# taddallas/HMSC

Measured on AMD Instinct MI355X. Metric: Gibbs sweeps/sec + Beta ESS/sec at ny=10k, ns=1k, nf=10; 1/2/4/8 MI355X, higher is better.
Workload: dtype f64; 1 GPU; synthetic probit JSDM ny=10000 ns=1000 nc=20 nf=10, 1 sample-level random level, updater GammaEta=FALSE, record every sweep; ny=10000, ns=1000, nc=20, nf=10, parallelism=1 independent chains, one per GPU

## Files before the change

### hmsc_amd/csrc/z_kernel.h

```cpp
#pragma once
#include <hip/hip_runtime.h>
#include <stdint.h>

#include "common.h"
#include "rng.h"
#include "record.h"
#include "z_tables.h"

namespace hmsc {

constexpr int Z_NSEG = 4;
struct ZSeg {
  int n, t;
};

struct ZArgs {
  const double* XEta;
  int ny, K, ns_loc, sp0, nt;
  ZSeg seg[Z_NSEG];
#ifdef HMSC_STAMPS
  int stamp_by, stamp_chunk;
#endif
  const double* BL;
  const double* iSigma;
  const int8_t* Ycode;
  const uint64_t* Ybits;
  const double* Yval;
  const int* fam;
  const double* Tr;
  double* Z;
  double* XZ_part;
  double* ZTr_part;
  Key key;
  uint32_t iter;
  const uint32_t* iter_dev;
  int noise_zero;
  int zprev_is_e;
  int mask_na;
  unsigned long long* kt;
  int gred_y0, gred_groups, gred_ntile, gred_nf, gred_Kmax;
  const double* gred_part;
  const double* gred_XX;
  double* gred_G;
  const double* logtab;
  const double* ztab;
  int pack_row;
  PackArgs pack;
};

constexpr int ZT_I = 64;
constexpr int ZT_J = 32;
constexpr int KMAX_Z = 128;
constexpr int ZT_LD = 65;

typedef double d4 __attribute__((ext_vector_type(4)));

__device__ __forceinline__ d4 mfma_f64(double a, double b, d4 c) {
  return __builtin_amdgcn_mfma_f64_16x16x4f64(a, b, c, 0, 0, 0);
}

__device__ __forceinline__ void wave_lds_sync() {
  __builtin_amdgcn_fence(__ATOMIC_RELEASE, "wavefront");
  __builtin_amdgcn_wave_barrier();
  __builtin_amdgcn_fence(__ATOMIC_ACQUIRE, "wavefront");
}

template <int N>
__device__ __forceinline__ double row_ror(double v) {
  const long long b = __double_as_longlong(v);
  const int lo = __builtin_amdgcn_update_dpp(0, (int)b, 0x120 + N, 0xF, 0xF, false);
  const int hi = __builtin_amdgcn_update_dpp(0, (int)(b >> 32), 0x120 + N, 0xF, 0xF, false);
  return __longlong_as_double(((long long)hi << 32) | (unsigned int)lo);
}
__device__ __forceinline__ double row_sum16(double v) {
  v += row_ror<8>(v);
  v += row_ror<4>(v);
  v += row_ror<2>(v);
  v += row_ror<1>(v);
  return v;
}

__device__ __noinline__ double z_probit_draw(double e, double sd, double isd, int code, double u, int noise_zero) {
  const double sg = code == 0 ? -1.0 : 1.0;
  if (code < 0 && noise_zero) return e;
  const double alpha = code < 0 ? -INFINITY : -sg * e * isd;
  return e + sd * sg * trunc_normal_lower(alpha, u);
}

constexpr int ZLOG_N = 64;
constexpr int ZLOG_W = 2;
inline void z_log_table(double* t) {
  for (int j = 0; j < ZLOG_N; ++j) {
    const long double c = 1.0L + (2 * j + 1) / 128.0L;
    t[ZLOG_W * j] = (double)(1.0L / c);
    t[ZLOG_W * j + 1] = (double)logl(c);
  }
}
HMSC_TABLE double kLog1pSeries[5] = {1.0 / 5.0, -1.0 / 4.0, 1.0 / 3.0, -1.0 / 2.0, 1.0};
__device__ __forceinline__ double log_tab(double x, const double* tab) {
  const int e = __builtin_amdgcn_frexp_exp(x) - 1;
  const double m2 = 2.0 * __builtin_amdgcn_frexp_mant(x);
  uint64_t b;
  __builtin_memcpy(&b, &m2, 8);
  const uint32_t hi = (uint32_t)(b >> 32);
  const int j = (int)((hi >> 14) & 63u);
  const uint64_t cb = (uint64_t)((hi & 0xFFFFC000u) | 0x2000u) << 32;
  double c;
  __builtin_memcpy(&c, &cb, 8);
  const double* tj = tab + ZLOG_W * j;
  const double r = (m2 - c) * tj[0];
  double P = kLog1pSeries[0];
#pragma unroll
  for (int k = 1; k < 5; ++k) P = fma_sc(P, r, kLog1pSeries[k]);
  const double de = (double)e;
  return fma(de, 0.6931471803691238, tj[1]) + fma(r, P, de * 1.9082149292705877e-10);
}

struct ZPair {
  double z0, z1;
};

#ifndef ZT_Q_LD_DEF
#define ZT_Q_LD_DEF 10
#endif
constexpr int ZT_E_LD = 10, ZT_Q_LD = ZT_Q_LD_DEF;
constexpr int ZT_E_SEG = ZT_E_MAX * ZT_E_PER_UNIT, ZT_Q_SEG = ZT_Q_MAX * ZT_Q_PER_UNIT;
constexpr int ZT_X_N = 64;
constexpr int ZT_OFF_E = 0, ZT_OFF_Q = ZT_E_SEG * ZT_E_LD, ZT_OFF_X = ZT_OFF_Q + ZT_Q_SEG * ZT_Q_LD;
constexpr int ZT_DOUBLES = ZT_OFF_X + ZT_X_N;
static_assert(ZT_E_NC % 2 == 0 && ZT_Q_NC % 2 == 0 && ZT_E_LD % 2 == 0 && ZT_Q_LD % 2 == 0 && ZT_E_LD >= ZT_E_NC &&
                  ZT_Q_LD >= ZT_Q_NC,
              "16-byte rows");
inline void z_draw_tables(double* t) {
  for (int i = 0; i < ZT_DOUBLES; ++i) t[i] = 0.0;
  for (int j = 0; j < ZT_E_SEG; ++j)
    for (int k = 0; k < ZT_E_NC; ++k) t[ZT_OFF_E + ZT_E_LD * j + k] = kZtErfcx[ZT_E_NC * j + k];
  for (int j = 0; j < ZT_Q_SEG; ++j)
    for (int k = 0; k < ZT_Q_NC; ++k) t[ZT_OFF_Q + ZT_Q_LD * j + k] = kZtQnormF[ZT_Q_NC * j + k];
  for (int i = 0; i < ZT_X_N; ++i) t[ZT_OFF_X + i] = kZtExp2[i];
}
typedef double zt_d2 __attribute__((ext_vector_type(2)));

template <int NC>
__device__ __forceinline__ double zt_poly(const double* row, double d) {
  const zt_d2* r2 = (const zt_d2*)row;
  zt_d2 c[NC / 2];
#pragma unroll
  for (int k = 0; k < NC / 2; ++k) c[k] = r2[k];
  double v = c[0][0];
  v = fma(v, d, c[0][1]);
#pragma unroll
  for (int k = 1; k < NC / 2; ++k) {
    v = fma(v, d, c[k][0]);
    v = fma(v, d, c[k][1]);
  }
  return v;
}

HMSC_TABLE double kZtExpPoly[6] = {1.0 / 120.0, 1.0 / 24.0, 1.0 / 6.0, 0.5, 1.0, 1.0};
template <bool IN_RANGE = false>
__device__ __forceinline__ double zt_erfc(double a, const double* zt) {
  const int j = IN_RANGE ? (int)(a * (double)ZT_E_PER_UNIT) : min((int)(a * (double)ZT_E_PER_UNIT), ZT_E_SEG - 1);
  const double d = a - ((double)j + 0.5) * (1.0 / ZT_E_PER_UNIT);
  const double* row = IN_RANGE ? (const double*)((const char*)(zt + ZT_OFF_E) +
                                                 __umul24((unsigned int)j, (unsigned int)(ZT_E_LD * sizeof(double))))
                               : zt + ZT_OFF_E + ZT_E_LD * j;
  const double cx = zt_poly<ZT_E_NC>(row, d);
  const double hi = a * a, lo = fma(a, a, -hi);
  const double kf = __builtin_rint(hi * -92.33248261689366);
  double r = fma(kf, -0.01083042469326756, -hi);
  r = fma(kf, -2.9815858269852933e-12, r) - lo;
  double p = kZtExpPoly[0];
#pragma unroll
  for (int k = 1; k < 6; ++k) p = fma_sc(p, r, kZtExpPoly[k]);
  const int ki = (int)kf;
  return __builtin_ldexp(p * zt[ZT_OFF_X + (ki & 63)], ki >> 6) * cx;
}

__device__ __forceinline__ double zt_qnorm_w(double p, double w, const double* zt) {
  const int j = max(0, min((int)(w * (double)ZT_Q_PER_UNIT), ZT_Q_SEG - 1));
  const double d = w - ((double)j + 0.5) * (1.0 / ZT_Q_PER_UNIT);
  return (2.0 * p - 1.0) * zt_poly<ZT_Q_NC>(zt + ZT_OFF_Q + ZT_Q_LD * j, d);
}

__device__ __forceinline__ ZPair z_probit_pair_tab(double e0, double e1, double sd0, double sd1, double isd0,
                                                double isd1, int c0, int c1, double u0, double u1, int noise_zero,
                                                const double* ltab, const double* zt) {
  const double sg0 = c0 == 0 ? -1.0 : 1.0, sg1 = c1 == 0 ? -1.0 : 1.0;
  const double al0 = c0 < 0 ? -INFINITY : -sg0 * e0 * isd0;
  const double al1 = c1 < 0 ? -INFINITY : -sg1 * e1 * isd1;
  double q0, q1;
  if (al0 > 25.0 || al1 > 25.0) {
    q0 = -trunc_normal_lower(al0, u0);
    q1 = -trunc_normal_lower(al1, u1);
  } else {
    const double a0 = fmin(fabs(al0) * 0.7071067811865476, 17.99);
    const double a1 = fmin(fabs(al1) * 0.7071067811865476, 17.99);
    const double r0 = 0.5 * zt_erfc(a0, zt), r1 = 0.5 * zt_erfc(a1, zt);
    const double s0 = 1.0 - r0, s1 = 1.0 - r1;
    const double p0 = u0 * (al0 < 0.0 ? s0 : r0), pc0 = fma(u0, al0 < 0.0 ? r0 : s0, 1.0 - u0);
    const double p1 = u1 * (al1 < 0.0 ? s1 : r1), pc1 = fma(u1, al1 < 0.0 ? r1 : s1, 1.0 - u1);
    const double w0 = -log_tab(4.0 * p0 * pc0, ltab), w1 = -log_tab(4.0 * p1 * pc1, ltab);
    q0 = zt_qnorm_w(p0, w0, zt);
    q1 = zt_qnorm_w(p1, w1, zt);
    if (w0 >= (double)ZT_Q_MAX || w1 >= (double)ZT_Q_MAX) {
      if (w0 >= (double)ZT_Q_MAX) q0 = qnorm_as241_tail_pq_t(p0, pc0, kLogSeries);
      if (w1 >= (double)ZT_Q_MAX) q1 = qnorm_as241_tail_pq_t(p1, pc1, kLogSeries);
    }
  }
  ZPair z;
  z.z0 = (c0 < 0 && noise_zero) ? e0 : e0 - sd0 * sg0 * q0;
  z.z1 = (c1 < 0 && noise_zero) ? e1 : e1 - sd1 * sg1 * q1;
  return z;
}
__device__ __forceinline__ double z_flip(double x, uint32_t f) {
  return __hiloint2double(__double2hiint(x) ^ (int)f, __double2loint(x));
}
__device__ __forceinline__ ZPair z_probit_pair_lean(double e0, double e1, uint32_t f0, uint32_t f1, double u0,
                                                    double u1, const double* ltab, const double* zt) {
  const double al0 = z_flip(e0, f0), al1 = z_flip(e1, f1);
  double q0, q1;
  if (al0 > 25.0 || al1 > 25.0) {
    q0 = -trunc_normal_lower(al0, u0);
    q1 = -trunc_normal_lower(al1, u1);
  } else {
    const double a0 = fmin(fabs(al0) * 0.7071067811865476, 17.99);
    const double a1 = fmin(fabs(al1) * 0.7071067811865476, 17.99);
    const double r0 = 0.5 * zt_erfc<true>(a0, zt), r1 = 0.5 * zt_erfc<true>(a1, zt);
    const double s0 = 1.0 - r0, s1 = 1.0 - r1;
    const double p0 = u0 * (al0 < 0.0 ? s0 : r0), pc0 = fma(u0, al0 < 0.0 ? r0 : s0, 1.0 - u0);
    const double p1 = u1 * (al1 < 0.0 ? s1 : r1), pc1 = fma(u1, al1 < 0.0 ? r1 : s1, 1.0 - u1);
    const double w0 = -log_tab(4.0 * p0 * pc0, ltab), w1 = -log_tab(4.0 * p1 * pc1, ltab);
    q0 = zt_qnorm_w(p0, w0, zt);
    q1 = zt_qnorm_w(p1, w1, zt);
    if (w0 >= (double)ZT_Q_MAX || w1 >= (double)ZT_Q_MAX) {
      if (w0 >= (double)ZT_Q_MAX) q0 = qnorm_as241_tail_pq_t(p0, pc0, kLogSeries);
      if (w1 >= (double)ZT_Q_MAX) q1 = qnorm_as241_tail_pq_t(p1, pc1, kLogSeries);
    }
  }
  ZPair z;
  z.z0 = e0 + z_flip(q0, f0);
  z.z1 = e1 + z_flip(q1, f1);
  return z;
}
__device__ __forceinline__ ZPair z_probit_pair(double e0, double e1, double sd0, double sd1, double isd0, double isd1,
                                            int c0, int c1, double u0, double u1, int noise_zero,
                                            const double* ltab) {
  const double sg0 = c0 == 0 ? -1.0 : 1.0, sg1 = c1 == 0 ? -1.0 : 1.0;
  const double al0 = c0 < 0 ? -INFINITY : -sg0 * e0 * isd0;
  const double al1 = c1 < 0 ? -INFINITY : -sg1 * e1 * isd1;
  double q0, q1;
  if (al0 > 25.0 || al1 > 25.0) {
    q0 = -trunc_normal_lower(al0, u0);
    q1 = -trunc_normal_lower(al1, u1);
  } else {
    const double h0 = al0 * 0.7071067811865476, h1 = al1 * 0.7071067811865476;
    const double a0 = fmin(fabs(h0), 40.0), a1 = fmin(fabs(h1), 40.0);
    const double t0 = 2.0 * rcp_pos(2.0 + a0), t1 = 2.0 * rcp_pos(2.0 + a1);
    const double x0 = 2.0 * t0 - 1.0, x1 = 2.0 * t1 - 1.0;
    double g0 = kErfcPoly[0], g1 = kErfcPoly[0];
#pragma unroll
    for (int k = 1; k < ERFC_NC; ++k) {
      g0 = fma_sc(g0, x0, kErfcPoly[k]);
      g1 = fma_sc(g1, x1, kErfcPoly[k]);
    }
    const double r0 = t0 * exp_small(fma(-a0, a0, g0)), r1 = t1 * exp_small(fma(-a1, a1, g1));
    const double p0 = u0 * (0.5 * (h0 < 0.0 ? 2.0 - r0 : r0));
    const double p1 = u1 * (0.5 * (h1 < 0.0 ? 2.0 - r1 : r1));
    const double pc0 = h0 < 0.0 ? fma(u0, 0.5 * r0, 1.0 - u0) : 1.0 - p0;
    const double pc1 = h1 < 0.0 ? fma(u1, 0.5 * r1, 1.0 - u1) : 1.0 - p1;
    const double w0 = -log_tab(4.0 * p0 * pc0, ltab), w1 = -log_tab(4.0 * p1 * pc1, ltab);
    const double y0 = w0 - 3.125, y1 = w1 - 3.125;
    double F0 = kQnormA[0], F1 = kQnormA[0];
#pragma unroll
    for (int k = 1; k < QNA_NC; ++k) {
      F0 = fma_sc(F0, y0, kQnormA[k]);
      F1 = fma_sc(F1, y1, kQnormA[k]);
    }
    q0 = (2.0 * p0 - 1.0) * F0;
    q1 = (2.0 * p1 - 1.0) * F1;
    if (w0 >= 6.25 || w1 >= 6.25) {
      const double sw0 = sqrt(fmax(w0, 6.25)) - 3.25, sw1 = sqrt(fmax(w1, 6.25)) - 3.25;
      double B0 = kQnormB[0], B1 = kQnormB[0];
#pragma unroll
      for (int k = 1; k < QNB_NC; ++k) {
        B0 = fma_sc(B0, sw0, kQnormB[k]);
        B1 = fma_sc(B1, sw1, kQnormB[k]);
      }
      if (w0 >= 6.25) q0 = w0 < 16.0 ? (2.0 * p0 - 1.0) * B0 : qnorm_as241_tail_pq_t(p0, pc0, kLogSeries);
      if (w1 >= 6.25) q1 = w1 < 16.0 ? (2.0 * p1 - 1.0) * B1 : qnorm_as241_tail_pq_t(p1, pc1, kLogSeries);
    }
  }
  ZPair z;
  z.z0 = (c0 < 0 && noise_zero) ? e0 : e0 - sd0 * sg0 * q0;
  z.z1 = (c1 < 0 && noise_zero) ? e1 : e1 - sd1 * sg1 * q1;
  return z;
}

__device__ __noinline__ double z_poisson_draw(double e, double sd, double y, double zprev, Uniform2 u,
                                              int noise_zero) {
  constexpr double R_NB = 1000.0, LOG_R = 6.907755278982137;
  double m, v;
  pg_moments(y + R_NB, zprev - LOG_R, &m, &v);
  const double omega = noise_zero ? m : fma(sqrt(v), qnorm_fast(u.a), m);
  const double prec = 1.0 / (sd * sd);
  const double sigz = 1.0 / (prec + omega);
  const double muz = fma(sigz, fma(prec, e - LOG_R, 0.5 * (y - R_NB)), LOG_R);
  return noise_zero ? muz : fma(sqrt(sigz), qnorm_fast(u.b), muz);
}

__device__ inline void g_reduce_body(const ZArgs& a, double* red) {
  const int lane = threadIdx.x & 63, w = threadIdx.x >> 6;
  const int K = a.K, Kmax = a.gred_Kmax, nf = a.gred_nf, nc = K - nf;
  const size_t stride = (size_t)Kmax * nf;
  for (int g = blockIdx.x; g < a.gred_groups; g += gridDim.x) {
    const int o = g * 64 + lane, k = o % K, h = o / K;
    double s = 0.0;
    if (o < K * nf) {
      const double* p = a.gred_part + k + (size_t)Kmax * h;
      int b = w;
      for (; b + 4 * 19 < a.gred_ntile; b += 4 * 20) {
        double x[20];
#pragma unroll
        for (int u = 0; u < 20; ++u) x[u] = p[stride * (b + 4 * u)];
#pragma unroll
        for (int u = 0; u < 20; ++u) s += x[u];
      }
      for (; b < a.gred_ntile; b += 4) s += p[stride * b];
    }
    __syncthreads();
    red[w * 64 + lane] = s;
    __syncthreads();
    if (w == 0 && o < K * nf) {
      const double v = (red[lane] + red[64 + lane]) + (red[128 + lane] + red[192 + lane]);
      a.gred_G[k + (size_t)Kmax * (nc + h)] = v;
      a.gred_G[(nc + h) + (size_t)Kmax * k] = v;
    }
    if (g == 0)
      for (int p = threadIdx.x; p < nc * nc; p += blockDim.x) a.gred_G[p % nc + (size_t)Kmax * (p / nc)] = a.gred_XX[p];
  }
}

constexpr int Z_ALL = 15;
constexpr int Z_NOSTORE = 16;
constexpr int ZT_TLD = 17;

#ifndef Z_MIN_BLOCKS
#define Z_MIN_BLOCKS 4
#endif
#ifdef HMSC_STAMPS
constexpr int Z_NSTAMP = 64;
extern __device__ unsigned long long g_zstamps[Z_NSTAMP];
#define Z_STAMP(i)                                                                 \
  do {                                                                             \
    unsigned long long t_;                                                         \
    __builtin_amdgcn_sched_barrier(0);                                             \
    asm volatile("s_memtime %0\n\ts_waitcnt lgkmcnt(0)" : "=s"(t_)::"memory");    \
    __builtin_amdgcn_sched_barrier(0);                                             \
    if (threadIdx.x == 0 && by == a.stamp_by && chunk == a.stamp_chunk && (i) < Z_NSTAMP) g_zstamps[(i)] = t_; \
  } while (0)
#define Z_STAMP_T(n, k) Z_STAMP(2 + 5 * (n) + (k))
#else
#define Z_STAMP(i) \
  do {             \
  } while (0)
#define Z_STAMP_T(n, k) \
  do {                  \
  } while (0)
#endif
template <bool DRAW, bool HAS_NA, int NKB, int MODE = Z_ALL, bool POIS = false, bool NORMAL = true, bool LEAN = false>
__global__ __launch_bounds__(256, NKB > 4 ? 2 : Z_MIN_BLOCKS) void z_wave_kernel(ZArgs a) {
  static_assert(!LEAN || (DRAW && !HAS_NA && !POIS && !NORMAL), "the lean pair draw: probit cells only, no NA");
  kernarg_warm<sizeof(ZArgs)>();
  extern __shared__ __attribute__((aligned(16))) double smem[];
  if (a.gred_y0 && blockIdx.y == 0) {
    g_reduce_body(a, smem);
    return;
  }
  if (a.pack_row && blockIdx.y == gridDim.y - 1) {
    pack_body(a.pack, blockIdx.x, gridDim.x);
    return;
  }
  const int by = (int)blockIdx.x;
  const int chunk = (int)blockIdx.y - a.gred_y0;
  const unsigned long long kt0 = a.kt ? kt_now() : 0ull;
  constexpr int K16 = 16 * NKB;
  const int K = a.K, K4 = (K + 3) & ~3;
  const int ny = a.ny;
  double* sBL = smem;
  double* sTr = sBL + K16 * ZT_J;
  double* sSd = sTr + ZT_J * a.nt;
  double* sIsd = sSd + ZT_J;
  int* sFam = (int*)(sIsd + ZT_J);
  double* sLog = (double*)(sFam + ZT_J);
  double* sZT = sLog + ZLOG_W * ZLOG_N;
  const int t = threadIdx.x, lane = t & 63, w = t >> 6, lm = lane & 15, lk = lane >> 4;
  const uint32_t iter = SWEEP_ITER(a);
  double* sT = sZT + ZT_DOUBLES + w * (ZT_J * ZT_TLD);
  const int j0 = by * ZT_J;
  const int n_tiles = (ny + ZT_I - 1) / ZT_I;
  int tb = 0, te = 0;
  {
    int c = chunk;
    bool found = false;
#pragma unroll
    for (int g = 0; g < Z_NSEG; ++g) {
      const int n = a.seg[g].n, tpc = a.seg[g].t;
      if (!found && c < n) {
        tb += c * tpc;
        te = min(n_tiles, tb + tpc);
        found = true;
      } else if (!found) {
        c -= n;
        tb += n * tpc;
      }
    }
  }
  Z_STAMP(0);
  constexpr int EC = NKB > 4 ? 16 : K16 / 4;
  uint64_t yw = 0;
  double xa[EC];
#pragma unroll
  for (int s4 = 0; s4 < EC; ++s4) xa[s4] = 0.0;
  auto load_e = [&](int i0t, int lmv, int lkv) {
    yw = a.Ybits[(size_t)by * ny + (i0t + lmv)];
    const double* xp = a.XEta + (i0t + lmv) + (size_t)ny * lkv;
#pragma unroll
    for (int s4 = 0; s4 < EC; ++s4) xa[s4] = xp[(size_t)ny * 4 * s4];
  };
  constexpr bool E_AHEAD = DRAW && ((NKB <= 2 && !HAS_NA) || NKB > 4);
  if (E_AHEAD && tb < te && tb * ZT_I + 16 * w < ny) load_e(tb * ZT_I + 16 * w, lm, lk);
  constexpr int NBL = K16 * ZT_J / 256, NZT = (ZT_DOUBLES + 255) / 256, NTR = 2;
  static_assert(ZLOG_W * ZLOG_N <= 256 && (ZLOG_W * ZLOG_N & (ZLOG_W * ZLOG_N - 1)) == 0,
                "the log table is staged by one load a thread, its index clamped by a mask");
  double vBL[NBL], vTr[NTR], vZT[NZT], vLog = 0.0;
#pragma unroll
  for (int u = 0; u < NBL; ++u) {
    const int p = t + 256 * u, k = p >> 5, j = j0 + (p & 31);
    vBL[u] = a.BL[(k < K && j < a.ns_loc) ? k + (size_t)K * j : 0];
  }
  auto tr_index = [&](int p) {
    const int j = j0 + (p & 31);
    return (p < ZT_J * a.nt && j < a.ns_loc) ? j + (size_t)a.ns_loc * (p >> 5) : (size_t)0;
  };
  if (a.nt > 0) {
#pragma unroll
    for (int u = 0; u < NTR; ++u) vTr[u] = a.Tr[tr_index(t + 256 * u)];
  }
  const int jt = (t < ZT_J && j0 + t < a.ns_loc) ? j0 + t : 0;
  const double vis = a.iSigma[jt];
  const int vfam = a.fam[jt];
  if (DRAW && (MODE & 2)) {
    vLog = a.logtab[t & (ZLOG_W * ZLOG_N - 1)];
#pragma unroll
    for (int u = 0; u < NZT; ++u) vZT[u] = a.ztab[min(t + 256 * u, ZT_DOUBLES - 1)];
  }
#pragma unroll
  for (int u = 0; u < NBL; ++u) {
    const int p = t + 256 * u, k = p >> 5, j = j0 + (p & 31);
    sBL[p] = (k < K && j < a.ns_loc) ? vBL[u] : 0.0;
  }
  if (a.nt > 0) {
#pragma unroll
    for (int u = 0; u < NTR; ++u) {
      const int p = t + 256 * u;
      if (p < ZT_J * a.nt) sTr[p] = (j0 + (p & 31) < a.ns_loc) ? vTr[u] : 0.0;
    }
    for (int p0 = NTR * 256; p0 < ZT_J * a.nt; p0 += NTR * 256) {
#pragma unroll
      for (int u = 0; u < NTR; ++u) vTr[u] = a.Tr[tr_index(p0 + t + 256 * u)];
#pragma unroll
      for (int u = 0; u < NTR; ++u) {
        const int p = p0 + t + 256 * u;
        if (p < ZT_J * a.nt) sTr[p] = (j0 + (p & 31) < a.ns_loc) ? vTr[u] : 0.0;
      }
    }
  }
  if (t < ZT_J) {
    const int j = j0 + t;
    const double is = (j < a.ns_loc) ? vis : 1.0;
    sSd[t] = 1.0 / sqrt(is);
    sIsd[t] = sqrt(is);
    sFam[t] = (j < a.ns_loc) ? vfam : 0;
  }
  if (DRAW && (MODE & 2)) {
    if (t < ZLOG_W * ZLOG_N) sLog[t] = vLog;
#pragma unroll
    for (int u = 0; u < NZT; ++u)
      if (t + 256 * u < ZT_DOUBLES) sZT[t + 256 * u] = vZT[u];
  }
  __syncthreads();
  Z_STAMP(1);

  d4 acc[NKB][2];
#pragma unroll
  for (int q = 0; q < NKB; ++q) acc[q][0] = acc[q][1] = d4{0.0, 0.0, 0.0, 0.0};

  for (int tile = tb; tile < te; ++tile) {
    const int i0 = tile * ZT_I + 16 * w;
    if (i0 >= ny) break;
    const bool more = DRAW && tile + 1 < te && i0 + ZT_I < ny;
    Z_STAMP_T(tile - tb, 0);
    auto ycode_of = [&](int m, int b) { return (int)((yw >> (4 * m + 2 * b)) & 3u) - 1; };
    if (DRAW) {
      if (!E_AHEAD) load_e(i0, lm, lk);
      d4 e0 = {0.0, 0.0, 0.0, 0.0}, e1 = {0.0, 0.0, 0.0, 0.0};
      const double* xp = a.XEta + (i0 + lm) + (size_t)ny * lk;
#pragma unroll
      for (int c0 = 0; c0 < K16 / 4; c0 += EC) {
        if (c0 > 0) {
#pragma unroll
          for (int s4 = 0; s4 < EC; ++s4) xa[s4] = xp[(size_t)ny * 4 * (c0 + s4)];
        }
#pragma unroll
        for (int s4 = 0; s4 < EC; ++s4) {
          const int k = 4 * (c0 + s4) + lk;
          if (MODE & 1) {
            e0 = mfma_f64(xa[s4], sBL[k * ZT_J + 2 * lm], e0);
            e1 = mfma_f64(xa[s4], sBL[k * ZT_J + 2 * lm + 1], e1);
          } else {
            e0[s4 & 3] += xa[s4];
          }
        }
      }
#pragma unroll
      for (int r = 0; r < 4; ++r) {
        sT[(2 * lm) * ZT_TLD + lk + 4 * r] = e0[r];
        sT[(2 * lm + 1) * ZT_TLD + lk + 4 * r] = e1[r];
      }
      wave_lds_sync();
    }
    Z_STAMP_T(tile - tb, 1);
    if constexpr (LEAN && (MODE & 2) != 0) {
      const int s = lm, i = i0 + s;
      double* const zl = a.Z + ((size_t)i + (size_t)ny * (size_t)(j0 + 4 * lk));
      double* const tl = sT + (4 * lk) * ZT_TLD + s;
      const uint32_t ctr0 = (uint32_t)i + (uint32_t)ny * (uint32_t)(((a.sp0 + j0) >> 2) + lk);
      const uint32_t yc = (((uint32_t)yw >> (8 * lk)) & 0xFFu) | ((((uint32_t)(yw >> 32) >> (8 * lk)) & 0xFFu) << 8);
      const bool inner = __builtin_amdgcn_readfirstlane(i0) + 16 <= ny && j0 + ZT_J <= a.ns_loc;
      U4 qw{0u, 0u, 0u, 0u};
#pragma unroll 1
      for (int c = 0; c < 4; ++c) {
        const int jc = 16 * (c >> 1) + 2 * (c & 1);
        if (!(c & 1))
          qw = philox4x32_10_wave_key(U4{ctr0 + (uint32_t)ny * (uint32_t)(4 * (c >> 1)), 0u, (uint32_t)S_Z, iter}, a.key);
        const double u0 = u32o((c & 1) ? qw.z : qw.x), u1 = u32o((c & 1) ? qw.w : qw.y);
        const uint32_t f0 = (yc << (30 - 4 * c)) & 0x80000000u, f1 = (yc << (28 - 4 * c)) & 0x80000000u;
        double* const tp = tl + jc * ZT_TLD;
        const int jj0 = 4 * lk + jc;
        const double e0 = tp[0], e1 = tp[ZT_TLD];
        const ZPair zp = z_probit_pair_lean(e0, e1, f0, f1, u0, u1, sLog, sZT);
        double z0 = zp.z0, z1 = zp.z1;
        double* const zc = zl + (size_t)ny * jc;
        if (inner) {
          if (!(MODE & Z_NOSTORE)) {
            zc[0] = z0;
            zc[ny] = z1;
          }
          tp[0] = z0;
          tp[ZT_TLD] = z1;
        } else {
          asm volatile("; z_edge_trip");
          const int ja = j0 + jj0;
          const bool in0 = i < ny && ja < a.ns_loc, in1 = i < ny && ja + 1 < a.ns_loc;
          if (!(MODE & Z_NOSTORE)) {
            if (in0) zc[0] = z0;
            if (in1) zc[ny] = z1;
          }
          tp[0] = in0 ? z0 : 0.0;
          tp[ZT_TLD] = in1 ? z1 : 0.0;
        }
      }
    } else {
      const int s = lm, i = i0 + s;
      U4 qw{0u, 0u, 0u, 0u};
#pragma unroll 1
      for (int c = 0; c < 4; ++c) {
        const int m = 8 * (c >> 1) + 2 * lk + (c & 1), ja = j0 + 2 * m;
        Uniform2 u{0.0, 0.0};
        if (DRAW) {
          if (!(c & 1))
            qw = philox4x32_10_wave_key(U4{(uint32_t)((size_t)i + (size_t)ny * (uint32_t)((a.sp0 + ja) >> 2)), 0u, (uint32_t)S_Z, iter}, a.key);
          u = (c & 1) ? Uniform2{u32o(qw.z), u32o(qw.w)} : Uniform2{u32o(qw.x), u32o(qw.y)};
        }
        if (DRAW && !POIS && (MODE & 2)) {
          const int cd0 = ycode_of(m, 0), cd1 = ycode_of(m, 1);
          const int jj0 = 2 * m, jj1 = 2 * m + 1;
          const bool in0 = i < ny && ja < a.ns_loc, in1 = i < ny && ja + 1 < a.ns_loc;
          const double e0 = sT[jj0 * ZT_TLD + s], e1 = sT[jj1 * ZT_TLD + s];
          const ZPair zp = z_probit_pair_tab(e0, e1, sSd[jj0], sSd[jj1], sIsd[jj0], sIsd[jj1], cd0, cd1, u.a, u.b,
                                             a.noise_zero, sLog, sZT);
          double z0 = zp.z0, z1 = zp.z1;
          if (NORMAL) {
            if (sFam[jj0] == 1 && cd0 >= 0 && in0) z0 = a.Yval[(size_t)i + (size_t)ny * ja];
            if (sFam[jj1] == 1 && cd1 >= 0 && in1) z1 = a.Yval[(size_t)i + (size_t)ny * (ja + 1)];
          }
          if (!(MODE & Z_NOSTORE)) {
            if (in0) a.Z[(size_t)i + (size_t)ny * ja] = z0;
            if (in1) a.Z[(size_t)i + (size_t)ny * (ja + 1)] = z1;
          }
          sT[jj0 * ZT_TLD + s] = in0 ? z0 : 0.0;
          sT[jj1 * ZT_TLD + s] = in1 ? z1 : 0.0;
          continue;
        }
#pragma unroll
        for (int b = 0; b < 2; ++b) {
          const int jj = 2 * m + b, j = ja + b;
          double z = 0.0;
          if (i < ny && j < a.ns_loc) {
            const size_t cell = (size_t)i + (size_t)ny * j;
            if (DRAW) {
              const int code = ycode_of(m, b);
              const double e = sT[jj * ZT_TLD + s];
              if (sFam[jj] == 1 && code >= 0)
                z = a.Yval[cell];
              else if (POIS && sFam[jj] == 3 && code >= 0)
                z = z_poisson_draw(e, sSd[jj], a.Yval[cell], a.zprev_is_e ? e : a.Z[cell],
                                   uniforms(a.key, (uint32_t)((size_t)i + (size_t)ny * (uint32_t)(a.sp0 + j)), 0,
                                            S_ZPOIS, iter),
                                   a.noise_zero);
              else if (MODE & 2)
                z = z_probit_draw(e, sSd[jj], sIsd[jj], code, b ? u.b : u.a, a.noise_zero);
              else
                z = e + (b ? u.b : u.a);
              if (!(MODE & Z_NOSTORE)) a.Z[cell] = z;
            } else {
              z = a.Z[cell];
            }
          }
          sT[jj * ZT_TLD + s] = z;
        }
      }
    }
    if (MODE & 8) {
      for (int tt = 0; tt < a.nt; ++tt) {
        const double* tr = sTr + tt * ZT_J;
        double v = 0.0;
#pragma unroll
        for (int c = 0; c < 4; ++c) {
          const int m = 4 * c + lk;
          v = fma(sT[(2 * m) * ZT_TLD + lm], tr[2 * m], v);
          v = fma(sT[(2 * m + 1) * ZT_TLD + lm], tr[2 * m + 1], v);
        }
        v += __shfl_xor(v, 16);
        v += __shfl_xor(v, 32);
        const int i = i0 + lm;
        if (lk == 0 && i < ny) a.ZTr_part[(size_t)by * ny * a.nt + i + (size_t)ny * tt] = v;
      }
    }
    wave_lds_sync();
    Z_STAMP_T(tile - tb, 2);
    Z_STAMP_T(tile - tb, 3);
    if ((MODE & 4) && NKB > 4) {
      double zz[4][2];
#pragma unroll
      for (int r = 0; r < 4; ++r) {
        const int ir = i0 + 4 * r + lk;
        zz[r][0] = sT[(2 * lm) * ZT_TLD + lk + 4 * r];
        zz[r][1] = sT[(2 * lm + 1) * ZT_TLD + lk + 4 * r];
        if (HAS_NA && a.mask_na) {
          const uint64_t w2 = a.Ybits[(size_t)by * ny + ir];
          if (((w2 >> (4 * lm)) & 3u) == 0) zz[r][0] = 0.0;
          if (((w2 >> (4 * lm + 2)) & 3u) == 0) zz[r][1] = 0.0;
        }
      }
      const double* xq = a.XEta + (i0 + lk) + (size_t)ny * lm;
#pragma unroll
      for (int q0 = 0; q0 < NKB; q0 += 4) {
        double xt[4][4];
#pragma unroll
        for (int r = 0; r < 4; ++r)
#pragma unroll
          for (int q = 0; q < 4; ++q) xt[r][q] = xq[4 * r + (size_t)ny * 16 * (q0 + q)];
#pragma unroll
        for (int r = 0; r < 4; ++r)
#pragma unroll
          for (int q = 0; q < 4; ++q) {
            acc[q0 + q][0] = mfma_f64(xt[r][q], zz[r][0], acc[q0 + q][0]);
            acc[q0 + q][1] = mfma_f64(xt[r][q], zz[r][1], acc[q0 + q][1]);
          }
      }
    } else if (MODE & 4) {
      double xt[4][NKB];
      const double* xq = a.XEta + (i0 + lk) + (size_t)ny * lm;
#pragma unroll
      for (int r = 0; r < 4; ++r)
#pragma unroll
        for (int q = 0; q < NKB; ++q) xt[r][q] = xq[4 * r + (size_t)ny * 16 * q];
#pragma unroll
      for (int r = 0; r < 4; ++r) {
        const int ir = i0 + 4 * r + lk;
        double z0 = sT[(2 * lm) * ZT_TLD + lk + 4 * r];
        double z1 = sT[(2 * lm + 1) * ZT_TLD + lk + 4 * r];
        if (HAS_NA && a.mask_na) {
          const uint64_t w2 = a.Ybits[(size_t)by * ny + ir];
          if (((w2 >> (4 * lm)) & 3u) == 0) z0 = 0.0;
          if (((w2 >> (4 * lm + 2)) & 3u) == 0) z1 = 0.0;
        }
#pragma unroll
        for (int q = 0; q < NKB; ++q) {
          acc[q][0] = mfma_f64(xt[r][q], z0, acc[q][0]);
          acc[q][1] = mfma_f64(xt[r][q], z1, acc[q][1]);
        }
      }
    }
    if (E_AHEAD && more) {
      int lmv = lm, lkv = lk;
      asm volatile("" : "+v"(lmv), "+v"(lkv));
      load_e(i0 + ZT_I, lmv, lkv);
    }
    wave_lds_sync();
    Z_STAMP_T(tile - tb, 4);
  }
  constexpr int QC = NKB > 4 ? 4 : NKB, KC = 16 * QC;
  double* sR = smem;
#pragma unroll
  for (int q0 = 0; q0 < NKB; q0 += QC) {
    __syncthreads();
    if (w > 0) {
#pragma unroll
      for (int q = 0; q < QC; ++q)
#pragma unroll
        for (int b = 0; b < 2; ++b)
#pragma unroll
          for (int rr = 0; rr < 4; ++rr)
            sR[((w - 1) * KC + 16 * q + lk + 4 * rr) * ZT_J + 2 * lm + b] = acc[q0 + q][b][rr];
    }
    __syncthreads();
    if (w == 0) {
      double* dst = a.XZ_part + (size_t)chunk * K * a.ns_loc;
#pragma unroll
      for (int q = 0; q < QC; ++q)
#pragma unroll
        for (int b = 0; b < 2; ++b)
#pragma unroll
          for (int rr = 0; rr < 4; ++rr) {
            const int kl = 16 * q + lk + 4 * rr, k = 16 * q0 + kl, jj = 2 * lm + b, j = j0 + jj;
            const double v = acc[q0 + q][b][rr] + sR[(0 * KC + kl) * ZT_J + jj] + sR[(1 * KC + kl) * ZT_J + jj] +
                             sR[(2 * KC + kl) * ZT_J + jj];
            if (k < K && j < a.ns_loc) dst[k + (size_t)K * j] = v;
          }
    }
  }
  if (w == 0 && a.kt && t == 0) kt_record(a.kt, iter, kt0);
}

inline int z_nkb(int K) {
  const int n = (K + 15) / 16;
  return n > 4 ? 8 : n;
}
inline int z_xeta_cols(int Kmax) { return 16 * z_nkb(Kmax); }

inline size_t z_smem_bytes(int K, int nt) {
  const size_t K16 = 16 * (size_t)z_nkb(K);
  const size_t body = K16 * ZT_J + (size_t)ZT_J * nt + 2 * ZT_J + ZT_J / 2 + ZLOG_W * (size_t)ZLOG_N + ZT_DOUBLES +
                      4 * (size_t)ZT_J * ZT_TLD;
  const size_t red = 3 * (K16 > 64 ? 64 : K16) * ZT_J;
  return (body > red ? body : red) * sizeof(double);
}

}
```

Before: 7709 sweeps/s.

## Software-pipeline LDS table lookups in lean probit pair with sched barriers

Splits the erfcx, exp, log and qnorm table lookups in the lean probit pair path into separate issue and finish steps. Sched barriers and register pins interleave the two lanes' LDS row loads with the other lane's polynomial arithmetic, so LDS latency is hidden within a thread. Lane 0's erfcx row fetch is also hoisted ahead of the call, and table rows are read as 16-byte vectors. The cost is higher register pressure and hand-fixed scheduling that can fight the compiler's own choices.

```diff
diff --git a/hmsc_amd/csrc/z_kernel.h b/hmsc_amd/csrc/z_kernel.h
--- a/hmsc_amd/csrc/z_kernel.h
+++ b/hmsc_amd/csrc/z_kernel.h
@@ -97,6 +97,34 @@
   }
 }
 HMSC_TABLE double kLog1pSeries[5] = {1.0 / 5.0, -1.0 / 4.0, 1.0 / 3.0, -1.0 / 2.0, 1.0};
+typedef double zt_d2 __attribute__((ext_vector_type(2)));
+struct ZLogRow {
+  double de, mc;
+  zt_d2 t;
+};
+__device__ __forceinline__ ZLogRow log_tab_issue(double x, const double* tab) {
+  const int e = __builtin_amdgcn_frexp_exp(x) - 1;
+  const double m2 = 2.0 * __builtin_amdgcn_frexp_mant(x);
+  uint64_t b;
+  __builtin_memcpy(&b, &m2, 8);
+  const uint32_t hi = (uint32_t)(b >> 32);
+  const int j = (int)((hi >> 14) & 63u);
+  const uint64_t cb = (uint64_t)((hi & 0xFFFFC000u) | 0x2000u) << 32;
+  double c;
+  __builtin_memcpy(&c, &cb, 8);
+  ZLogRow l;
+  l.t = *(const zt_d2*)(tab + ZLOG_W * j);
+  l.mc = m2 - c;
+  l.de = (double)e;
+  return l;
+}
+__device__ __forceinline__ double log_tab_finish(const ZLogRow& l) {
+  const double r = l.mc * l.t[0];
+  double P = kLog1pSeries[0];
+#pragma unroll
+  for (int k = 1; k < 5; ++k) P = fma_sc(P, r, kLog1pSeries[k]);
+  return fma(l.de, 0.6931471803691238, l.t[1]) + fma(r, P, l.de * 1.9082149292705877e-10);
+}
 __device__ __forceinline__ double log_tab(double x, const double* tab) {
   const int e = __builtin_amdgcn_frexp_exp(x) - 1;
   const double m2 = 2.0 * __builtin_amdgcn_frexp_mant(x);
@@ -139,7 +167,6 @@
     for (int k = 0; k < ZT_Q_NC; ++k) t[ZT_OFF_Q + ZT_Q_LD * j + k] = kZtQnormF[ZT_Q_NC * j + k];
   for (int i = 0; i < ZT_X_N; ++i) t[ZT_OFF_X + i] = kZtExp2[i];
 }
-typedef double zt_d2 __attribute__((ext_vector_type(2)));
 
 template <int NC>
 __device__ __forceinline__ double zt_poly(const double* row, double d) {
@@ -216,23 +243,130 @@
 __device__ __forceinline__ double z_flip(double x, uint32_t f) {
   return __hiloint2double(__double2hiint(x) ^ (int)f, __double2loint(x));
 }
-__device__ __forceinline__ ZPair z_probit_pair_lean(double e0, double e1, uint32_t f0, uint32_t f1, double u0,
-                                                    double u1, const double* ltab, const double* zt) {
-  const double al0 = z_flip(e0, f0), al1 = z_flip(e1, f1);
+#define Z_FENCE() __builtin_amdgcn_sched_barrier(0)
+#define Z_PHASE(x)         \
+  do {                     \
+    Z_FENCE();             \
+    asm volatile("" : "+v"(x)); \
+  } while (0)
+template <int NC>
+__device__ __forceinline__ void zt_row_issue(const double* row, zt_d2 (&c)[NC / 2]) {
+  const zt_d2* r2 = (const zt_d2*)row;
+#pragma unroll
+  for (int k = 0; k < NC / 2; ++k) c[k] = r2[k];
+}
+template <int NC>
+__device__ __forceinline__ double zt_row_poly(const zt_d2 (&c)[NC / 2], double d) {
+  double v = c[0][0];
+  v = fma(v, d, c[0][1]);
+#pragma unroll
+  for (int k = 1; k < NC / 2; ++k) {
+    v = fma(v, d, c[k][0]);
+    v = fma(v, d, c[k][1]);
+  }
+  return v;
+}
+__device__ __forceinline__ const double* zt_erfcx_row(int j, const double* zt) {
+  return (const double*)((const char*)(zt + ZT_OFF_E) + __umul24((unsigned int)j, (unsigned int)(ZT_E_LD * sizeof(double))));
+}
+struct ZLead {
+  double al, a;
+  int j;
+  zt_d2 c[ZT_E_NC / 2];
+};
+__device__ __forceinline__ void z_lead_issue(ZLead& L, double e0, uint32_t f0, const double* zt) {
+  L.al = z_flip(e0, f0);
+  L.a = fmin(fabs(L.al) * 0.7071067811865476, 17.99);
+  L.j = (int)(L.a * (double)ZT_E_PER_UNIT);
+  zt_row_issue<ZT_E_NC>(zt_erfcx_row(L.j, zt), L.c);
+}
+struct ZExpPart {
+  double p, x;
+  int ki;
+};
+__device__ __forceinline__ ZExpPart zt_exp_issue(double a, const double* zt) {
+  const double hi = a * a, lo = fma(a, a, -hi);
+  const double kf = __builtin_rint(hi * -92.33248261689366);
+  ZExpPart x;
+  x.ki = (int)kf;
+  x.x = zt[ZT_OFF_X + (x.ki & 63)];
+  double r = fma(kf, -0.01083042469326756, -hi);
+  r = fma(kf, -2.9815858269852933e-12, r) - lo;
+  double p = kZtExpPoly[0];
+#pragma unroll
+  for (int k = 1; k < 6; ++k) p = fma_sc(p, r, kZtExpPoly[k]);
+  x.p = p;
+  return x;
+}
+__device__ __forceinline__ ZPair z_probit_pair_lean(double e0, double e1, uint32_t f0, uint32_t f1, uint32_t uw0,
+                                                    uint32_t uw1, const ZLead& L, const double* ltab,
+                                                    const double* zt) {
+  const double al0 = L.al, al1 = z_flip(e1, f1);
   double q0, q1;
   if (al0 > 25.0 || al1 > 25.0) {
-    q0 = -trunc_normal_lower(al0, u0);
-    q1 = -trunc_normal_lower(al1, u1);
+    q0 = -trunc_normal_lower(al0, u32o(uw0));
+    q1 = -trunc_normal_lower(al1, u32o(uw1));
   } else {
-    const double a0 = fmin(fabs(al0) * 0.7071067811865476, 17.99);
-    const double a1 = fmin(fabs(al1) * 0.7071067811865476, 17.99);
-    const double r0 = 0.5 * zt_erfc<true>(a0, zt), r1 = 0.5 * zt_erfc<true>(a1, zt);
-    const double s0 = 1.0 - r0, s1 = 1.0 - r1;
+    const double a0 = L.a;
+    double a1 = fmin(fabs(al1) * 0.7071067811865476, 17.99);
+    ZExpPart x0 = zt_exp_issue(a0, zt);
+    double d0 = a0 - ((double)L.j + 0.5) * (1.0 / ZT_E_PER_UNIT);
+    Z_PHASE(d0);
+    const double cx0 = zt_row_poly<ZT_E_NC>(L.c, d0);
+    Z_PHASE(x0.p);
+    double ex0 = __builtin_ldexp(x0.p * x0.x, x0.ki >> 6) * cx0;
+    Z_PHASE(a1);
+    ZExpPart x1 = zt_exp_issue(a1, zt);
+    const int j1 = (int)(a1 * (double)ZT_E_PER_UNIT);
+    const double* rowB = zt_erfcx_row(j1, zt);
+    double d1 = a1 - ((double)j1 + 0.5) * (1.0 / ZT_E_PER_UNIT);
+    Z_FENCE();
+    zt_d2 cB[ZT_E_NC / 2];
+    zt_row_issue<ZT_E_NC>(rowB, cB);
+    Z_PHASE(ex0);
+    const double u0 = u32o(uw0);
+    const double r0 = 0.5 * ex0;
+    const double s0 = 1.0 - r0;
     const double p0 = u0 * (al0 < 0.0 ? s0 : r0), pc0 = fma(u0, al0 < 0.0 ? r0 : s0, 1.0 - u0);
+    Z_PHASE(x1.p);
+    const double px1 = x1.p * x1.x;
+    ZLogRow l0 = log_tab_issue(4.0 * p0 * pc0, ltab);
+    Z_PHASE(d1);
+    const double cx1 = zt_row_poly<ZT_E_NC>(cB, d1);
+    const double u1 = u32o(uw1);
+    const double r1 = 0.5 * (__builtin_ldexp(px1, x1.ki >> 6) * cx1);
+    const double s1 = 1.0 - r1;
     const double p1 = u1 * (al1 < 0.0 ? s1 : r1), pc1 = fma(u1, al1 < 0.0 ? r1 : s1, 1.0 - u1);
-    const double w0 = -log_tab(4.0 * p0 * pc0, ltab), w1 = -log_tab(4.0 * p1 * pc1, ltab);
-    q0 = zt_qnorm_w(p0, w0, zt);
-    q1 = zt_qnorm_w(p1, w1, zt);
+    ZLogRow l1 = log_tab_issue(4.0 * p1 * pc1, ltab);
+    Z_PHASE(l0.mc);
+    const double w0 = -log_tab_finish(l0);
+    const int jq0 = max(0, min((int)(w0 * (double)ZT_Q_PER_UNIT), ZT_Q_SEG - 1));
+    double dq0 = w0 - ((double)jq0 + 0.5) * (1.0 / ZT_Q_PER_UNIT);
+    zt_d2 cF0[ZT_Q_NC / 2];
+    zt_row_issue<ZT_Q_NC>(zt + ZT_OFF_Q + ZT_Q_LD * jq0, cF0);
+    Z_PHASE(l1.mc);
+    const double w1 = -log_tab_finish(l1);
+    const int jq1 = max(0, min((int)(w1 * (double)ZT_Q_PER_UNIT), ZT_Q_SEG - 1));
+    double dq1 = w1 - ((double)jq1 + 0.5) * (1.0 / ZT_Q_PER_UNIT);
+    zt_d2 cF1[ZT_Q_NC / 2];
+    const zt_d2* rowF1 = (const zt_d2*)(zt + ZT_OFF_Q + ZT_Q_LD * jq1);
+    Z_PHASE(dq0);
+    double v = cF0[0][0];
+    v = fma(v, dq0, cF0[0][1]);
+    Z_PHASE(v);
+    cF1[0] = rowF1[0];
+    Z_FENCE();
+#pragma unroll
+    for (int k = 1; k < ZT_Q_NC / 2; ++k) {
+      v = fma(v, dq0, cF0[k][0]);
+      v = fma(v, dq0, cF0[k][1]);
+      Z_PHASE(v);
+      cF1[k] = rowF1[k];
+      Z_FENCE();
+    }
+    q0 = (2.0 * p0 - 1.0) * v;
+    Z_PHASE(dq1);
+    q1 = (2.0 * p1 - 1.0) * zt_row_poly<ZT_Q_NC>(cF1, dq1);
     if (w0 >= (double)ZT_Q_MAX || w1 >= (double)ZT_Q_MAX) {
       if (w0 >= (double)ZT_Q_MAX) q0 = qnorm_as241_tail_pq_t(p0, pc0, kLogSeries);
       if (w1 >= (double)ZT_Q_MAX) q1 = qnorm_as241_tail_pq_t(p1, pc1, kLogSeries);
@@ -392,6 +526,7 @@
   double* sSd = sTr + ZT_J * a.nt;
   double* sIsd = sSd + ZT_J;
   int* sFam = (int*)(sIsd + ZT_J);
+  static_assert(ZT_J % 4 == 0 && ZLOG_W == 2 && (ZLOG_W * ZLOG_N) % 2 == 0, "16-byte aligned table rows");
   double* sLog = (double*)(sFam + ZT_J);
   double* sZT = sLog + ZLOG_W * ZLOG_N;
   const int t = threadIdx.x, lane = t & 63, w = t >> 6, lm = lane & 15, lk = lane >> 4;
@@ -542,14 +677,16 @@
 #pragma unroll 1
       for (int c = 0; c < 4; ++c) {
         const int jc = 16 * (c >> 1) + 2 * (c & 1);
-        if (!(c & 1))
-          qw = philox4x32_10_wave_key(U4{ctr0 + (uint32_t)ny * (uint32_t)(4 * (c >> 1)), 0u, (uint32_t)S_Z, iter}, a.key);
-        const double u0 = u32o((c & 1) ? qw.z : qw.x), u1 = u32o((c & 1) ? qw.w : qw.y);
         const uint32_t f0 = (yc << (30 - 4 * c)) & 0x80000000u, f1 = (yc << (28 - 4 * c)) & 0x80000000u;
         double* const tp = tl + jc * ZT_TLD;
         const int jj0 = 4 * lk + jc;
+        if (!(c & 1))
+          qw = philox4x32_10_wave_key(U4{ctr0 + (uint32_t)ny * (uint32_t)(4 * (c >> 1)), 0u, (uint32_t)S_Z, iter}, a.key);
+        const uint32_t uw0 = (c & 1) ? qw.z : qw.x, uw1 = (c & 1) ? qw.w : qw.y;
         const double e0 = tp[0], e1 = tp[ZT_TLD];
-        const ZPair zp = z_probit_pair_lean(e0, e1, f0, f1, u0, u1, sLog, sZT);
+        ZLead lead;
+        z_lead_issue(lead, e0, f0, sZT);
+        const ZPair zp = z_probit_pair_lean(e0, e1, f0, f1, uw0, uw1, lead, sLog, sZT);
         double z0 = zp.z0, z1 = zp.z1;
         double* const zc = zl + (size_t)ny * jc;
         if (inner) {
```

Result: no change. 7750 sweeps/s (median of 2 runs) (+0.5%).
